# DeepLearningZ/chanamq

Measured on AMD Instinct MI355X. Metric: msgs/sec (whole node) + p50 publish→deliver latency, 1 KB payload, 1/2/4/8 GPUs, higher is better.
Workload: dtype uint8 (AMQP wire bytes; no floating-point compute)

## Files before the change

### csrc/kernels/dataplane.hip

```cpp
#include "dp_state.h"

#define INVALID 0xffffffffu
#define FNV64_BASIS 0xcbf29ce484222325ULL
#define FNV64_PRIME 0x100000001b3ULL

DEV u32 lane_id() { return __lane_id(); }
DEV u64 lanemask_lt() {
  u32 l = __lane_id();
  return l ? ((~0ull) >> (64 - l)) : 0ull;
}
DEV u32 be16(const u8* p) { return (u32(p[0]) << 8) | u32(p[1]); }
DEV u32 be32(const u8* p) {
  return (u32(p[0]) << 24) | (u32(p[1]) << 16) | (u32(p[2]) << 8) | u32(p[3]);
}
DEV u64 be64(const u8* p) { return (u64(be32(p)) << 32) | u64(be32(p + 4)); }
DEV void wr16(u8* p, u32 v) { p[0] = u8(v >> 8); p[1] = u8(v); }
DEV void wr32(u8* p, u32 v) { p[0] = u8(v >> 24); p[1] = u8(v >> 16); p[2] = u8(v >> 8); p[3] = u8(v); }
DEV void wr64(u8* p, u64 v) { wr32(p, u32(v >> 32)); wr32(p + 4, u32(v)); }
DEV u32 align16(u32 x) { return (x + 15u) & ~15u; }

DEV u64 exch_hash(u32 vhost, const u8* name, u32 n) {
  u64 h = FNV64_BASIS ^ (u64(vhost) * 0x9E3779B97F4A7C15ULL);
  for (u32 i = 0; i < n; ++i) { h ^= name[i]; h *= FNV64_PRIME; }
  return h;
// ... 157 lines not shown
DEV void release_msg(const DS& d, u32 msg) {
  if (msg == INVALID) return;
  i32 old = atomicSub(&d.msgs[msg].refcnt, 1);
  if (old == 1) {
    MsgEnt& m = d.msgs[msg];
    if (m.log_off & COLD_BIT) {
      atomicAdd((unsigned long long*)&d.cold_live[((m.log_off & ~COLD_BIT) >> COLD_SEG_SHIFT) % COLD_SEGS],
                (unsigned long long)(-(i64)m.slot_bytes));
    } else if (m.log_off & SPILL_BIT) {
      spill_free(d, m.log_off, m.slot_bytes);
    } else {
      u64 blk = (m.log_off / d.log_block) % d.n_log_blocks;
      atomicAdd((unsigned long long*)&d.log_live[blk], (unsigned long long)(-(i64)m.slot_bytes));
      atomicAdd((unsigned long long*)d.live_bytes, (unsigned long long)(-(i64)m.slot_bytes));
    }
    u32 slot = atomicAdd(d.msg_free_top, 1u);
    d.msg_free[slot] = msg;
    atomicAdd(&d.ctr->n_freed, 1u);
  }
}

DEV void wave_release(const DS& d, u32 msg, bool valid) {
  bool freed = false, spilled = false;
  u64 blk = 0;
  i64 sb = 0;
  if (valid && msg != INVALID) {
    i32 old = atomicSub(&d.msgs[msg].refcnt, 1);
    if (old == 1) {
      freed = true;
      const u64 lo = d.msgs[msg].log_off;
      sb = d.msgs[msg].slot_bytes;
      spilled = (lo & (SPILL_BIT | COLD_BIT)) != 0;
      if (lo & COLD_BIT)
        atomicAdd((unsigned long long*)&d.cold_live[((lo & ~COLD_BIT) >> COLD_SEG_SHIFT) % COLD_SEGS],
                  (unsigned long long)(-sb));
      else if (spilled) spill_free(d, lo, (u32)sb);
      else blk = (lo / d.log_block) % d.n_log_blocks;
    }
  }
  u64 fm = __ballot(freed);
  if (!fm) return;
  u32 nf;
  u32 pos = wave_reserve(d.msg_free_top, freed, &nf);
  if (freed) d.msg_free[pos] = msg;
  i64 tot = wave_sum64(freed && !spilled ? sb : 0);
  if (lane_id() == __ffsll((unsigned long long)fm) - 1) {
    atomicAdd(&d.ctr->n_freed, nf);
    if (tot) atomicAdd((unsigned long long*)d.live_bytes, (unsigned long long)(-tot));
  }
  wave_add_i64(d.log_live, blk, -sb, freed && !spilled);
}

DEV u64 snowflake_id(u64 pos, u32 group) {
  const u64 ms = pos >> ID_SLOT_BITS;
  const u64 worker = (u64)(group & (1023 / ID_WORKERS)) * ID_WORKERS + ((pos >> 12) & (ID_WORKERS - 1));
  return (ms << 22) | (worker << 12) | (pos & 4095);
}

struct Words { u32 eff; u32 count; };
DEV Words words_of(const u8* s, u32 n) {
  Words w;
  if (n == 0) { w.eff = 0; w.count = 1; return w; }
  u32 e = n;
  while (e > 0 && s[e - 1] == '.') --e;
  w.eff = e;
  if (e == 0) { w.count = 0; return w; }
  u32 c = 1;
  for (u32 i = 0; i < e; ++i) c += (s[i] == '.');
  w.count = c;
  return w;
}
DEV u32 word_len(const u8* s, u32 off, u32 eff) {
  u32 i = off;
  while (i < eff && s[i] != '.') ++i;
  return i - off;
}
DEV bool word_eq(const u8* a, u32 al, const u8* b, u32 bl) {
  if (al != bl) return false;
  for (u32 i = 0; i < al; ++i)
    if (a[i] != b[i]) return false;
  return true;
}
DEV bool topic_match(const u8* pat, u32 plen, const u8* key, u32 klen, bool hash_wild) {
  Words pw = words_of(pat, plen), kw = words_of(key, klen);
  u32 pend = pw.eff + 1, kend = kw.eff + 1;
  u32 p = pw.count ? 0 : pend, k = kw.count ? 0 : kend;
  u32 sp = INVALID, sk = 0;
  while (k < kend) {
    u32 kl = word_len(key, k, kw.eff);
    if (p < pend) {
      u32 pl = word_len(pat, p, pw.eff);
      bool is_hash = hash_wild && pl == 1 && pat[p] == '#';
      bool is_star = pl == 1 && pat[p] == '*';
      if (is_hash) { p += pl + 1; sp = p; sk = k; continue; }
      if (is_star || word_eq(pat + p, pl, key + k, kl)) { p += pl + 1; k += kl + 1; continue; }
    }
    if (sp != INVALID) {
      sk += word_len(key, sk, kw.eff) + 1;
      k = sk;
      p = sp;
      continue;
    }
    return false;
  }
  while (p < pend) {
    u32 pl = word_len(pat, p, pw.eff);
    if (hash_wild && pl == 1 && pat[p] == '#') { p += pl + 1; continue; }
    return false;
  }
  return true;
}

struct DeltaHead { u32 nrec, ndirty, nchunk, pad; };
struct DeltaRec { u64 dst; u32 len; u32 chunk0; };
#define DELTA_REC_MAX 1024
DEV void apply_deltas(const DS& d, const u8* buf, u32 tid, u32 nt, DeltaRec* lrec) {
  const DeltaHead h = *(const DeltaHead*)buf;
  const DeltaRec* recs = (const DeltaRec*)(buf + sizeof(DeltaHead));
  const u32* dirty = (const u32*)(recs + h.nrec);
  const uint4* data = (const uint4*)((const u8*)dirty + ((4u * h.ndirty + 15u) & ~15u));
  for (u32 r = tid; r < h.nrec; r += nt) lrec[r] = recs[r];
  __syncthreads();
  for (u32 i = tid; i < h.nchunk; i += nt) {
    u32 lo = 0, hi = h.nrec;
    while (hi - lo > 1) {
      const u32 mid = (lo + hi) >> 1;
      if (lrec[mid].chunk0 <= i) lo = mid; else hi = mid;
    }
    const DeltaRec r = lrec[lo];
    const u32 off = (i - r.chunk0) * 16u;
    const u32 n = r.len - off < 16u ? r.len - off : 16u;
    const uint4 v = data[i];
    u8* dst = (u8*)(uintptr_t)(r.dst + off);
    const u32 w[4] = {v.x, v.y, v.z, v.w};
    if (((uintptr_t)dst & 3) == 0 && (n & 3) == 0) {
      for (u32 k = 0; k < n / 4; ++k) ((u32*)dst)[k] = w[k];
    } else {
      for (u32 k = 0; k < n; ++k) dst[k] = (u8)(w[k >> 2] >> (8 * (k & 3)));
    }
  }
  __syncthreads();
  for (u32 k = tid; k < h.ndirty; k += nt) {
    const u32 ch = dirty[k];
    if (atomicExch(&d.ch_dirty[ch], 1u) == 0) d.dirty_list[atomicAdd(d.n_dirty, 1u)] = ch;
  }
  __threadfence();
  __syncthreads();
}
__global__ __launch_bounds__(1024) void k_apply_deltas(DS d, const u8* buf) {
  __shared__ DeltaRec lrec[DELTA_REC_MAX];
  apply_deltas(d, buf, threadIdx.x, 1024, lrec);
}

__global__ __launch_bounds__(64) void k_h2d_wait(DS d) {
  const u64 sig = d.in->h2d_sig, sig2 = d.in->h2d_sig2;
  if (!sig) return;
  const u32 lim = d.in->h2d_polls ? d.in->h2d_polls : (1u << 24);
  if (threadIdx.x == 0)
    for (u32 it = 0; it < lim; ++it) {
      if (__hip_atomic_load((const i64*)sig, __ATOMIC_RELAXED, __HIP_MEMORY_SCOPE_SYSTEM) == 0 &&
          (!sig2 || __hip_atomic_load((const i64*)sig2, __ATOMIC_RELAXED, __HIP_MEMORY_SCOPE_SYSTEM) == 0))
        break;
      __builtin_amdgcn_s_sleep(4);
    }
  __syncthreads();
  __builtin_amdgcn_fence(__ATOMIC_ACQUIRE, "");
}

__global__ __launch_bounds__(1024) void k_stage(DS d) {
  __shared__ u32 lds[1024 / 64 + 1];
  __shared__ StepIn s_in;
  __shared__ DeltaRec lrec[DELTA_REC_MAX];
  const u32 tid = threadIdx.x;
  if (tid == 0) {
    s_in = *d.in_h;
    *d.in = s_in;
  }
  __syncthreads();
  if (s_in.delta_bytes) apply_deltas(d, d.delta_h, tid, 1024, lrec);
  const u32 nseg = s_in.nseg;
  {
    u32* c = (u32*)d.ctr;
    for (u32 k = tid; k < sizeof(Counters) / 4; k += 1024)
      if (k * 4 < offsetof(Counters, log_head)) c[k] = 0;
    if (tid == 0) {
      d.ctr->n_grow = 0; d.tot[TS_NMOVE] = 0; d.tot[TS_NDEFER] = 0; d.tot[TS_TTL_BUDGET] = 0;
      d.tot[TS_NDGET] = 0;
      d.tot[TS_SPILL_USED] = 0;
      d.ctr->spill_moved = 0;
      d.ctr->n_ref = 0; d.ctr->gath_off = 0; d.ctr->ref_bytes = 0;
      *d.egress_budget = 0;
    }
    const u32 nunp = s_in.nunp;
    for (u32 k = tid; k < nunp; k += 1024) {
      const u32 c = d.unpause_req[k];
      if (c < d.c_max) d.conn_paused[c] = 0;
    }
  }
  u32 total = 0;
  u32 cl0 = 0, len0 = 0;
  for (u32 k = tid; k < nseg; k += 1024) {
    const SegIn sg = d.segs_h[k];
    ((SegIn*)d.segs)[k] = sg;
    const u32 cl = d.carry_len[sg.conn];
    if (k == tid) { cl0 = cl; len0 = sg.len; }
    total += align16(cl + sg.len + 32);
  }
  u32 all_t;
  block_scan<1024>(total, lds, all_t);
  if (tid == 0) d.tot[15] = all_t;
  if (all_t > d.work_cap) return;
  u32 run = 0;
  for (u32 b0 = 0; b0 < nseg; b0 += 1024) {
    const u32 k = b0 + tid;
    u32 cl = 0, len = 0, v = 0;
    if (k < nseg) {
      if (b0 == 0) {
        cl = cl0;
        len = len0;
      } else {
        const SegIn sg = d.segs_h[k];
        cl = d.carry_len[sg.conn];
        len = sg.len;
      }
      v = align16(cl + len + 32);
    }
    u32 all;
    __syncthreads();
    const u32 o = block_scan<1024>(v, lds, all);
    if (k < nseg) { d.seg_total[k] = cl + len; d.seg_start[k] = run + o; }
    run += all;
  }
}

struct FInfo { u32 type, ch, size; bool complete, valid_hdr; };

DEV FInfo frame_at(const u8* b, u32 p, u32 L, u32 fmax) {
  FInfo f;
  f.complete = false;
  f.valid_hdr = false;
  f.type = 0; f.ch = 0; f.size = 0;
  if (p + 7 > L) return f;
  f.type = b[p];
  f.ch = be16(b + p + 1);
  f.size = be32(b + p + 3);
  bool tok = f.type == 1 || f.type == 2 || f.type == 3 || f.type == 8;
  bool sok = fmax == 0 || f.size + 8 <= fmax;
  f.valid_hdr = tok && sok;
  if (f.valid_hdr && (u64)p + 8 + f.size <= L) f.complete = (b[p + 7 + f.size] == 0xCE);
  return f;
}

DEV i32 chan_lookup(const DS& d, u32 conn, u32 ch) {
  const u32* m = d.chmap + (u64)conn * d.chmap_size;
  u32 mask = d.chmap_size - 1;
  u32 h = (ch * 0x9E3779B1u) >> 7;
  for (u32 i = 0; i < d.chmap_size; ++i) {
    u32 e = m[(h + i) & mask];
    if (e == 0) return -1;
    if ((e >> 16) == ch && (e & 0x8000u)) return (i32)(conn * d.chpc + (e & 0x7fffu));
  }
  return -1;
}

DEV u32 zero_bytes(u32 v) { return ~(((v & 0x7F7F7F7Fu) + 0x7F7F7F7Fu) | v | 0x7F7F7F7Fu); }
DEV u32 type_nibble(u32 v) {
  const u32 h = (zero_bytes(v & 0xFCFCFCFCu) & ~zero_bytes(v)) | zero_bytes(v ^ 0x08080808u);
  return (((h >> 7) * 0x00204081u) >> 21) & 0xFu;
}
DEV u32 cand_bits(uint4 A, uint4 B, u32 fm) {
  const u32 w[6] = {A.x, A.y, A.z, A.w, B.x, B.y};
  u32 m = 0;
#pragma unroll
  for (int i = 0; i < 4; ++i) {
    u32 h = type_nibble(w[i]);
    while (h) {
      const u32 k = __ffs(h) - 1;
      h &= h - 1;
      const u32 v = k == 0 ? __builtin_amdgcn_alignbyte(w[i + 1], w[i], 3)
                           : __builtin_amdgcn_alignbyte(w[i + 2], w[i + 1], k - 1);
      const u32 sz = __builtin_bswap32(v);
      if (fm == 0 || sz <= fm - 8) m |= 1u << (4 * i + k);
    }
  }
  return m;
}
DEV u32 cand_word(const u8* w16, u32 fm) {
  const uint4* q = (const uint4*)w16;
  return cand_bits(q[0], q[1], fm);
}

#define FS_MARK(k) \
  do { if (tid == 0 && d.dbg) d.dbg[(u64)s * 16 + (k)] = __builtin_amdgcn_s_memrealtime(); } while (0)
constexpr u32 FS_AM_MAX = 8192;
constexpr u32 FS_STAGE = 72u << 10;
constexpr u32 FS_CAND_STAGED = 6144;
constexpr u32 fs_cand_bytes(u32 cmax, u32 amw) { return cmax * 4 * 2 + (cmax > amw ? cmax : amw) * 2 + cmax * 2 + cmax; }
constexpr u32 FS_POOL_STAGED = FS_STAGE + fs_cand_bytes(FS_CAND_STAGED, FS_STAGE / 16);
constexpr u32 FS_POOL_FULL = fs_cand_bytes(CAND_MAX, FS_AM_MAX);
constexpr u32 FS_POOL = ((FS_POOL_STAGED > FS_POOL_FULL ? FS_POOL_STAGED : FS_POOL_FULL) + 15) & ~15u;
static_assert(FS_POOL <= 156u << 10, "k_frame_scan LDS pool");
#define FS_NT 1024
DEV bool big_publish(const DS& d, u32 msize, u32 hsize, u64 bsz, u32 fmax) {
  const u64 fb = fmax > 8 ? fmax - 8 : 0;
  const u64 nb = bsz == 0 ? 0 : (fb ? (bsz + fb - 1) / fb : 1);
  return (u64)msize + 8 + hsize + 8 + bsz + 8 * nb > d.carry_cap;
}

DEV uint4 shift_pair(uint4 a, uint4 b, u32 sh) {
  const u32 q = sh >> 2, r = sh & 3;
  const bool q2 = (q & 2) != 0, q1 = (q & 1) != 0;
  const u32 s0 = q2 ? a.z : a.x, s1 = q2 ? a.w : a.y, s2 = q2 ? b.x : a.z;
  const u32 s3 = q2 ? b.y : a.w, s4 = q2 ? b.z : b.x, s5 = q2 ? b.w : b.y;
  const u32 w0 = q1 ? s1 : s0, w1 = q1 ? s2 : s1, w2 = q1 ? s3 : s2, w3 = q1 ? s4 : s3, w4 = q1 ? s5 : s4;
  if (!r) return make_uint4(w0, w1, w2, w3);
  return make_uint4(__builtin_amdgcn_alignbyte(w1, w0, r), __builtin_amdgcn_alignbyte(w2, w1, r),
                    __builtin_amdgcn_alignbyte(w3, w2, r), __builtin_amdgcn_alignbyte(w4, w3, r));
}
DEV uint4 seg_word(const u8* C, u32 cl, const u8* N, u32 c) {
  const u32 b0 = c * 16;
  if (b0 + 16 <= cl) return *(const uint4*)(C + b0);
  if (b0 >= cl) {
    const u32 o = b0 - cl, k = o >> 4, sh = o & 15;
    const uint4 a = ((const uint4*)N)[k];
    return sh ? shift_pair(a, ((const uint4*)N)[k + 1], sh) : a;
  }
// ... 2126 lines not shown
}
DEV u32 enqueue_one(const DS& d, u32 src, u32 i, u32 n, PersistRec* pr, u32 hs_ntiles) {
  const u32* kk = d.pair_k[src];
  const u32 rb = d.rank_bits;
  u32 q = kk[i] >> rb;
  u32 p = d.pair_v[src][i];
  u32 first = hs_ntiles ? d.hist_scan[q << rb] : d.q_first[q];
  return enqueue_at(d, q, p, i - first, (i + 1 == n) || (kk[i + 1] >> rb) != q, pr);
}

DEV void plan_queue(const DS& d, u32 q, u64 cnt);
DEV void ring_plan_one(const DS& d, u32 src, u32 hs_ntiles, u32 i, u32 n) {
  const u32* kk = d.pair_k[src];
  const u32 rb = d.rank_bits;
  const u32 q = kk[i] >> rb;
  if (i + 1 < n && (kk[i + 1] >> rb) == q) return;
  const u32 first = hs_ntiles ? d.hist_scan[q << rb] : d.q_first[q];
  plan_queue(d, q, (u64)(i - first) + 1);
}
DEV void plan_queue(const DS& d, u32 q, u64 cnt) {
  const u64 head = d.q_head[q], tail = d.q_tail[q];
  d.q_enq_tail[q] = tail;
  const u64 mask = d.q_ring_mask[q], cap = mask + 1;
  const u64 need = tail - head + cnt;
  if (need <= cap) return;
  const u64 limit = d.q_max_cap[q] ? d.q_max_cap[q] : d.ring_pool;
  u64 want = cap;
  while (want < 2 * need && want * 2 <= limit) want *= 2;
  if (want <= cap) return;
  unsigned long long* top = (unsigned long long*)d.ring_top;
  u64 off = __hip_atomic_load(top, __ATOMIC_RELAXED, __HIP_MEMORY_SCOPE_AGENT);
  while (true) {
    if (off + want > d.ring_pool) return;
    u64 prev = atomicCAS(top, off, off + want);
    if (prev == off) break;
    off = prev;
  }
  RingMove mv;
  mv.q = q; mv.pad = 0;
  mv.old_off = d.q_ring_off[q]; mv.old_mask = mask;
  mv.new_off = off; mv.new_mask = want - 1;
  mv.head = head; mv.tail = tail;
  const u32 mi = atomicAdd(&d.tot[TS_NMOVE], 1u);
  d.moves[mi] = mv;
  d.q_ring_off[q] = off;
  d.q_ring_mask[q] = want - 1;
  const u32 gi = atomicAdd(&d.ctr->n_grow, 1u);
  if (gi < GROW_MAX) d.grow_h[gi] = mv;
  __threadfence();
}

__global__ __launch_bounds__(256) void k_ring_plan(DS d, u32 src, u32 hs_ntiles) {
  __shared__ u32 s_last;
  const u32 n = d.tot[TS_PAIR_N];
  u32 nb = (n + 255) / 256;
  if (nb > gridDim.x) nb = gridDim.x;
  if (blockIdx.x >= nb) return;
  for (u32 i = blockIdx.x * 256 + threadIdx.x; i < n; i += gridDim.x * 256) ring_plan_one(d, src, hs_ntiles, i, n);
  __builtin_amdgcn_fence(__ATOMIC_RELEASE, "workgroup");
  __syncthreads();
  if (threadIdx.x == 0) s_last = atomicAdd(&d.tot[TS_RP_TICKET], 1u) == nb - 1;
  __syncthreads();
  if (!s_last) return;
  __builtin_amdgcn_fence(__ATOMIC_ACQUIRE, "agent");
  if (threadIdx.x == 0) d.tot[TS_RP_TICKET] = 0;
  const u32 nm = d.tot[TS_NMOVE];
  for (u32 m = 0; m < nm; ++m) {
    const RingMove mv = d.moves[m];
    for (u64 pos = mv.head + threadIdx.x; pos < mv.tail; pos += 256)
      d.ring[mv.new_off + (pos & mv.new_mask)] = d.ring[mv.old_off + (pos & mv.old_mask)];
  }
}

__global__ void k_enqueue(DS d, u32 src, u32 hs_ntiles) {
  const u32 n = d.tot[TS_PAIR_N];
  const u32 stride = gridDim.x * blockDim.x;
  for (u32 b = blockIdx.x * blockDim.x; b < n; b += stride) {
    const u32 i = b + threadIdx.x;
    PersistRec pr;
    pr.msg = INVALID;
    u32 drop = i < n ? enqueue_one(d, src, i, n, &pr, hs_ntiles) : INVALID;
    wave_release(d, drop, drop != INVALID);
    if (drop != INVALID) atomicAdd(&d.ctr->n_ring_full, 1u);
    if (d.persist) {
      bool want = pr.msg != INVALID;
      u32 k = wave_reserve(&d.ctr->n_persist, want);
      if (want && k < d.persist_max) d.prec[k] = pr;
    }
  }
}

DEV void plan_rings_block(const DS& d, const u32* hscan, u32 n, u32 D, u32 tid, u32 nt) {
  const u32 rb = d.rank_bits;
  for (u32 q = tid; q < d.q_max && (q << rb) < D; q += nt) {
    const u32 first = __hip_atomic_load(&hscan[q << rb], __ATOMIC_RELAXED, __HIP_MEMORY_SCOPE_AGENT);
    const u32 nx = ((q + 1) << rb) < D
                       ? __hip_atomic_load(&hscan[(q + 1) << rb], __ATOMIC_RELAXED, __HIP_MEMORY_SCOPE_AGENT)
                       : n;
    if (nx > first) plan_queue(d, q, nx - first);
  }
  __syncthreads();
  const u32 nm = __hip_atomic_load(&d.tot[TS_NMOVE], __ATOMIC_RELAXED, __HIP_MEMORY_SCOPE_AGENT);
  if (!nm) return;
  __builtin_amdgcn_fence(__ATOMIC_ACQUIRE, "agent");
  for (u32 m = 0; m < nm; ++m) {
    const RingMove mv = d.moves[m];
    for (u64 pos = mv.head + tid; pos < mv.tail; pos += nt)
      d.ring[mv.new_off + (pos & mv.new_mask)] = d.ring[mv.old_off + (pos & mv.old_mask)];
  }
}

template <int DB>
__global__ __launch_bounds__(RsNt<DB>::v) void k_rs_hist_plan(DS d, const u32* keys, const u32* np, u32* hist,
                                                             u32* hscan, u32* ticket, u32 ntiles) {
  constexpr u32 NT = RsNt<DB>::v, D = 1u << DB;
  __shared__ u32 cnt[D];
  __shared__ u32 lds[NT / 64 + 1];
  __shared__ u32 s_last;
  u32 tid = threadIdx.x, t = blockIdx.x;
  const u32 n = *np;
  u32 T = (n + SORT_TILE - 1) / SORT_TILE;
  if (T > ntiles) T = ntiles;
  if (T == 0) {
    return;
  }
  if (t >= T) return;
  bool last = false;
  for (; t < T; t += gridDim.x) {
    for (u32 k = tid; k < D; k += NT) cnt[k] = 0;
    __syncthreads();
    const u32 base = t * SORT_TILE;
    for (u32 j = 0; j < SORT_TILE / NT; ++j) {
      const u32 i = base + j * NT + tid;
      if (i < n) atomicAdd(&cnt[keys[i] & (D - 1)], 1u);
    }
    __syncthreads();
    for (u32 k = tid; k < D; k += NT)
      __hip_atomic_store(&hist[t * D + k], cnt[k], __ATOMIC_RELAXED, __HIP_MEMORY_SCOPE_AGENT);
    __builtin_amdgcn_fence(__ATOMIC_RELEASE, "workgroup");
    __syncthreads();
    if (tid == 0) s_last = atomicAdd(ticket, 1u) == T - 1;
    __syncthreads();
    last = last || s_last;
  }
  if (!last) return;
  __builtin_amdgcn_fence(__ATOMIC_ACQUIRE, "agent");
  if (tid == 0) *ticket = 0;
  rs_offsets<DB>(hist, hscan, T, lds);
  __builtin_amdgcn_fence(__ATOMIC_RELEASE, "workgroup");
  __syncthreads();
  plan_rings_block(d, hscan, n, D, tid, NT);
}

template <int DB>
__global__ __launch_bounds__(256) void k_rs_scatter_enq(DS d, const u32* kin, const u32* vin, const u32* np,
                                                       const u32* hscan) {
  constexpr u32 D = 1u << DB, CH = SORT_TILE / 256;
  __shared__ u32 wc[4][D];
  const u32 tid = threadIdx.x, w = tid >> 6, lane = tid & 63;
  const u32 n = *np, rb = d.rank_bits;
  const u64 lt = lanemask_lt();
  for (u32 t = blockIdx.x; t * SORT_TILE < n; t += gridDim.x) {
    const u32 base = t * SORT_TILE;
    __syncthreads();
    for (u32 i = tid; i < 4 * D; i += 256) ((u32*)wc)[i] = 0;
    __syncthreads();
    const u32 wbase = base + w * (SORT_TILE / 4);
    u32 key[CH], val[CH];
    u64 pe[CH];
#pragma unroll
    for (u32 c = 0; c < CH; ++c) {
      const u32 i = wbase + c * 64 + lane;
      key[c] = i < n ? kin[i] : 0u;
      val[c] = i < n ? vin[i] : 0u;
    }
#pragma unroll
    for (u32 c = 0; c < CH; ++c) {
      const bool valid = wbase + c * 64 + lane < n;
      const u32 dg = key[c] & (D - 1);
      u64 peers = __ballot(valid);
#pragma unroll
      for (u32 bb = 0; bb < DB; ++bb) {
        const u64 m = __ballot((dg >> bb) & 1);
        peers &= ((dg >> bb) & 1) ? m : ~m;
      }
      pe[c] = peers;
      if (valid && ((peers & lt) == 0)) wc[w][dg] += __popcll(peers);
      __builtin_amdgcn_wave_barrier();
    }
    __syncthreads();
    for (u32 dg = tid; dg < D; dg += 256) {
      u32 run = hscan[t * D + dg];
      for (u32 ww = 0; ww < 4; ++ww) { const u32 x = wc[ww][dg]; wc[ww][dg] = run; run += x; }
    }
    __syncthreads();
    u32 pos[CH];
#pragma unroll
    for (u32 c = 0; c < CH; ++c) {
      const bool valid = wbase + c * 64 + lane < n;
      const u32 dg = key[c] & (D - 1);
      const u32 basepos = ((volatile u32*)wc[w])[dg];
      pos[c] = basepos + __popcll(pe[c] & lt);
      __builtin_amdgcn_wave_barrier();
      if (valid && ((pe[c] & lt) == 0)) ((volatile u32*)wc[w])[dg] = basepos + __popcll(pe[c]);
      __builtin_amdgcn_wave_barrier();
    }
    EnqLoad el[CH];
    u32 first[CH], nx[CH];
#pragma unroll
    for (u32 c = 0; c < CH; ++c) {
      const bool valid = wbase + c * 64 + lane < n;
      const u32 q = key[c] >> rb;
      first[c] = valid ? hscan[q << rb] : 0u;
      nx[c] = valid ? (((q + 1) << rb) < D ? hscan[(q + 1) << rb] : n) : 0u;
      el[c] = valid ? enq_load(d, q, val[c]) : EnqLoad{};
    }
#pragma unroll
    for (u32 c = 0; c < CH; ++c) {
      const bool valid = wbase + c * 64 + lane < n;
      PersistRec pr;
      pr.msg = INVALID;
      u32 drop = INVALID;
      if (valid) drop = enq_store(d, el[c], key[c] >> rb, pos[c] - first[c], pos[c] + 1 == nx[c], &pr);
      wave_release(d, drop, drop != INVALID);
      if (drop != INVALID) atomicAdd(&d.ctr->n_ring_full, 1u);
      if (d.persist) {
        const bool want = pr.msg != INVALID;
        const u32 k = wave_reserve(&d.ctr->n_persist, want);
        if (want && k < d.persist_max) d.prec[k] = pr;
      }
    }
  }
}

DEV bool wants_record(const DS& d, u32 msg, u32 q, bool valid) {
  return d.persist && valid && msg != INVALID && d.q_durable[q] && (d.msgs[msg].flags & MF_PERSIST);
}
DEV void consumed_rec_at(const DS& d, u32 msg, u32 q, u64 qpos, u32 kind, u32 k) {
  ConsumedRec r;
  r.msg_id = (i64)d.msgs[msg].msg_id;
  r.qpos = qpos;
  r.q = q;
  r.kind = kind;
  r.pad[0] = r.pad[1] = 0;
  d.crec[k] = r;
}
DEV void link_consumed(const DS& d, u32 msg, u32 q, u32 kind, bool valid) {
  if (d.links && valid && msg != INVALID && kind <= 2u) {
    const u32 ow = d.q_link_owner[q];
    if (ow) {
      const u32 k = atomicAdd(&d.lk_cnt[ow - 1], 1u);
      if (k < d.lk_cap) {
        AckRec a;
        a.tq = q;
        a.pad = 0;
        a.xid = d.msgs[msg].msg_id;
        d.lk_send[(u64)(ow - 1) * d.lk_cap + k] = a;
      }
    }
  }
}
DEV void wave_consumed(const DS& d, u32 msg, u32 q, u64 qpos, u32 kind, bool valid) {
  link_consumed(d, msg, q, kind, valid);
  if (!d.persist) return;
  bool want = wants_record(d, msg, q, valid);
  u32 k = wave_reserve(&d.ctr->n_consumed, want);
  if (want && k < d.persist_max) consumed_rec_at(d, msg, q, qpos, kind, k);
}


#define MS_MAX 256
struct MsLds {
  u64 up[MS_MAX];
  u32 rq[MS_MAX];
  u32 wc[4];
  u32 rc[4];
  u32 rbase;
  u32 n, nb;
  unsigned long long ovf_a, ovf_r;
};
DEV void chan_advance_one(const DS& d, u32 ch, u32 tid, u32 lane, u32 w, u32* s_first, u32* s_done, MsLds& ms);
__global__ __launch_bounds__(256) void k_chan_advance(DS d) {
  __shared__ u32 s_first[4];
  __shared__ u32 s_done[4];
  __shared__ MsLds ms;
  const u32 tid = threadIdx.x, lane = lane_id(), w = tid >> 6;
  const u32 nd = *d.n_dirty;
  for (u32 wv = blockIdx.x; wv < nd; wv += gridDim.x) chan_advance_one(d, d.dirty_list[wv], tid, lane, w, s_first,
                                                                        s_done, ms);
}

DEV void collect_settles(const DS& d, u32 ch, u32 tid, u32 lane, u32 w, MsLds& ms) {
  const u32 lo = d.ch_mlo[ch], hi = d.ch_mhi[ch];
  if (tid == 0) { ms.n = 0; ms.nb = 0; ms.ovf_a = 0; ms.ovf_r = 0; }
  __syncthreads();
  if (lo == INVALID) return;
  for (u32 base = lo; base <= hi; base += 256) {
    const u32 i = base + tid;
    bool take = false;
    Ack a;
    a.tag = 0; a.kind = 0; a.requeue = 0;
    if (i <= hi) {
      a = d.acks[i];
      take = a.chslot == ch && a.multiple;
    }
    const bool rq = (a.kind != CK_ACK) && a.requeue;
    const u64 m = __ballot(take);
    if (lane == 0) ms.wc[w] = (u32)__popcll(m);
    __syncthreads();
    u32 pos = ms.n + (u32)__popcll(m & lanemask_lt());
    for (u32 k = 0; k < w; ++k) pos += ms.wc[k];
    if (take) {
      if (pos < MS_MAX) { ms.up[pos] = a.tag; ms.rq[pos] = rq; }
      else atomicMax(rq ? &ms.ovf_r : &ms.ovf_a, (unsigned long long)a.tag);
    }
    __syncthreads();
    if (tid == 0) ms.n += ms.wc[0] + ms.wc[1] + ms.wc[2] + ms.wc[3];
    __syncthreads();
  }
  if (tid == 0) {
    const u32 n = ms.n < MS_MAX ? ms.n : MS_MAX;
    u64 top = 0;
    u32 nb = 0;
    for (u32 k = 0; k < n; ++k)
      if (ms.up[k] > top) { ms.up[nb] = ms.up[k]; ms.rq[nb] = ms.rq[k]; ++nb; top = ms.up[k]; }
    const u64 oa = ms.ovf_a, orq = ms.ovf_r;
    const u64 om = oa > orq ? oa : orq;
    if (om > top && nb < MS_MAX) { ms.up[nb] = om; ms.rq[nb] = orq > oa; ++nb; }
    ms.nb = nb;
    d.ch_mlo[ch] = INVALID;
    d.ch_mhi[ch] = 0;
  }
  __syncthreads();
}

DEV u32 ca_reserve(const DS& d, u32 n) {
  const u32 lim = d.persist_max - d.deliv_max - (d.persist_max >> 2) - 64u;
  u32 cur = *(volatile u32*)&d.ctr->n_consumed;
  while (true) {
    if (cur + n > lim) return INVALID;
    const u32 prev = atomicCAS(&d.ctr->n_consumed, cur, cur + n);
    if (prev == cur) return cur;
    cur = prev;
  }
}

DEV void chan_advance_one(const DS& d, u32 ch, u32 tid, u32 lane, u32 w, u32* s_first, u32* s_done, MsLds& ms) {
  collect_settles(d, ch, tid, lane, w, ms);
  const u32 nb = ms.nb;
  const u64 head = d.ch_uhead[ch], nt = d.ch_next_tag[ch];
  const u64 aup = d.ch_ack_upto[ch], rup = d.ch_req_upto[ch];
  USlot* win = d.uwin + (u64)ch * (d.ucap_mask + 1);
  bool contiguous = true;
  bool deferred = false;
  u64 newhead = head;
  u32 manual_done = 0;
  for (u64 t0 = head; t0 < nt; t0 += 256) {
    const u64 t = t0 + tid;
    const bool valid = t < nt;
    u32 st = US_FREE;
    USlot u;
    u.state = US_FREE; u.msg = INVALID; u.q = 0; u.cons = 0; u.qpos = 0; u.expire_ms = 0;
    if (valid) {
      u = win[(t - 1) & d.ucap_mask];
      st = u.state;
      if (st == US_PENDING) {
        if (t <= aup) st = US_ACKED;
        else if (t <= rup) st = US_REQUEUE;
        else
          for (u32 k = 0; k < nb; ++k)
            if (t <= ms.up[k]) { st = ms.rq[k] ? US_REQUEUE : US_ACKED; break; }
      }
    }
    const bool acked = valid && st == US_ACKED;
    const bool req = valid && st == US_REQUEUE;
    u32 rec_k = INVALID;
    const bool want_rec = wants_record(d, u.msg, u.q, acked || req);
    if (d.persist) {
      const u64 rm = __ballot(want_rec);
      if (lane == 0) ms.rc[w] = (u32)__popcll(rm);
      __syncthreads();
      if (tid == 0) {
        const u32 tot = ms.rc[0] + ms.rc[1] + ms.rc[2] + ms.rc[3];
        ms.rbase = deferred ? INVALID : (tot ? ca_reserve(d, tot) : 0u);
      }
      __syncthreads();
      if (ms.rbase == INVALID) deferred = true;
      if (!deferred) {
        rec_k = ms.rbase + (u32)__popcll(rm & lanemask_lt());
        for (u32 k = 0; k < w; ++k) rec_k += ms.rc[k];
      }
    }
    if (deferred) {
      if (valid && (st == US_ACKED || st == US_REQUEUE) && st != u.state) win[(t - 1) & d.ucap_mask].state = st;
      contiguous = false;
      continue;
    }
    u32 rtot;
    u32 ri = wave_reserve(d.req_n, req, &rtot);
    bool req_ok = req && ri < d.req_max;
    if (req_ok) {
      ReqItem r;
      r.q = u.q; r.msg = u.msg; r.qpos = u.qpos; r.expire_ms = u.expire_ms;
      d.req[ri] = r;
    }
    wave_add_u32(d.req_q_n, u.q, 1u, req_ok);
    link_consumed(d, u.msg, u.q, acked ? 0u : (req_ok ? 4u : 2u), acked || req);
    if (want_rec) consumed_rec_at(d, u.msg, u.q, u.qpos, acked ? 0u : (req_ok ? 4u : 2u), rec_k);
    wave_release(d, u.msg, acked || (req && !req_ok));
    wave_sub_u32(d.cons_unacked, u.cons, 1u, acked || req);
    manual_done += __popcll(__ballot(acked || req));
    if (lane == 0 && rtot) atomicAdd(&d.ctr->n_requeue, rtot);
    if (acked || req) st = US_DONE;
    if (valid && st != u.state) win[(t - 1) & d.ucap_mask].state = st;
    if (contiguous) {
      const u64 notdone = __ballot(valid && st != US_DONE);
      const u32 nvalid = (u32)__popcll(__ballot(valid));
      if (lane == 0) {
        s_first[w] = notdone ? (u32)(__ffsll((unsigned long long)notdone) - 1) : 64u;
        s_done[w] = nvalid;
      }
      __syncthreads();
      u32 adv = 0;
      bool stop = false;
      for (u32 k = 0; k < 4 && !stop; ++k) {
        if (s_first[k] < 64) { adv += s_first[k]; stop = true; }
        else adv += s_done[k];
      }
      newhead += adv;
      if (stop) contiguous = false;
      __syncthreads();
    }
  }
  if (lane == 0 && manual_done) atomicSub(&d.ch_unacked[ch], manual_done);
// ... 1548 lines not shown
```

### csrc/kernels/engine.hip

```cpp
#include <pybind11/pybind11.h>
#include <pybind11/numpy.h>
#include <pybind11/stl.h>

#include <chrono>
#include <algorithm>
#include <deque>
#include <functional>
#include <map>
#include <memory>
#include <mutex>
#include <condition_variable>
#include <thread>
#include <stdexcept>
#include <string>
#include <vector>

#include <hsa/amd_hsa_signal.h>
#include <hsa/hsa.h>
#include <hsa/hsa_ext_amd.h>
#include <rocprofiler-sdk-roctx/roctx.h>

#include "dataplane.hip"
#include "xchg_host.h"
#include "xchg_rccl.h"
// ... 2158 lines not shown
      if (t == HSA_DEVICE_TYPE_GPU) c->gpus.push_back(a);
      else if (t == HSA_DEVICE_TYPE_CPU) c->cpus.push_back(a);
      return HSA_STATUS_SUCCESS;
    }, &ctx);
    if ((int)ctx.gpus.size() <= device_ || ctx.cpus.empty()) throw std::runtime_error("HSA agents not found");
    {
      u64 f = 0;
      if (hsa_system_get_info(HSA_SYSTEM_INFO_TIMESTAMP_FREQUENCY, &f) != HSA_STATUS_SUCCESS || !f) f = 100000000ull;
      spin_ticks_ = f / 500;
      block_ticks_ = f / 1000;
    }
    gpu_agent_ = ctx.gpus[device_];
    cpu_agent_ = ctx.cpus[0];
    uint32_t mask = 0;
    if (hsa_amd_memory_copy_engine_status(cpu_agent_, gpu_agent_, &mask) != HSA_STATUS_SUCCESS || !mask)
      throw std::runtime_error("no SDMA engine available for device -> host copies");
    u32 pick = 0;
    if (sdma_pref_ >= 0 && (mask >> sdma_pref_) & 1u) pick = (u32)sdma_pref_;
    else if ((mask >> 1) & 1u) pick = 1;
    else while (!((mask >> pick) & 1u)) ++pick;
    sdma_engine_ = (hsa_amd_sdma_engine_id_t)(1u << pick);
    sdma_engine2_ = (hsa_amd_sdma_engine_id_t)0;
    if (sdma_split_ > 1)
      for (u32 c : {2u, 3u, 0u})
        if (c != pick && ((mask >> c) & 1u)) { sdma_engine2_ = (hsa_amd_sdma_engine_id_t)(1u << c); break; }
    tail_engine_ = sdma_engine_;
    for (u32 c : {2u, 3u, 0u})
      if (c != pick && ((mask >> c) & 1u) && (1u << c) != (u32)sdma_engine2_) {
        tail_engine_ = (hsa_amd_sdma_engine_id_t)(1u << c);
        break;
      }
    ing_engine_ = (hsa_amd_sdma_engine_id_t)0;
    for (u32 c : {0u, 3u, 2u, 1u})
      if (((mask >> c) & 1u) && (1u << c) != (u32)sdma_engine_ && (1u << c) != (u32)sdma_engine2_ &&
          (1u << c) != (u32)tail_engine_) {
        ing_engine_ = (hsa_amd_sdma_engine_id_t)(1u << c);
        break;
      }
    if (!ing_engine_) ing_engine_ = tail_engine_;
    ing_engine2_ = (hsa_amd_sdma_engine_id_t)0;
    if (h2d_split_cfg_)
      for (u32 c : {3u, 2u})
        if (((mask >> c) & 1u) && (1u << c) != (u32)ing_engine_ && (1u << c) != (u32)sdma_engine_ &&
            (1u << c) != (u32)sdma_engine2_ && (1u << c) != (u32)tail_engine_) {
          ing_engine2_ = (hsa_amd_sdma_engine_id_t)(1u << c);
          break;
        }
    for (int e = 0; e < EGRESS_SLOTS; ++e)
      if (hsa_signal_create(0, 0, nullptr, &sdma_sig_[e]) != HSA_STATUS_SUCCESS ||
          hsa_signal_create(0, 0, nullptr, &tail_sig_[e]) != HSA_STATUS_SUCCESS ||
          hsa_signal_create(0, 0, nullptr, &gate_sig_[e]) != HSA_STATUS_SUCCESS)
        throw std::runtime_error("hsa_signal_create failed");
  }

  void drain_egress() {
    for (int e = 0; e < EGRESS_SLOTS; ++e) {
      sdma_wait(e);
      if (d2h_issued_[e]) HIPCHECK(hipEventSynchronize(ev_d2h_[e]));
    }
  }

  void sync() {
    HIPCHECK(hipStreamSynchronize(s_h2d_));
    if (s_h2d_alt_) HIPCHECK(hipStreamSynchronize(s_h2d_alt_));
    HIPCHECK(hipStreamSynchronize(s_pre_));
    HIPCHECK(hipStreamSynchronize(s_ing_));
    HIPCHECK(hipStreamSynchronize(s_comp_));
    HIPCHECK(hipStreamSynchronize(s_d2h_));
  }

  py::dict host_times(bool reset) {
    static const char* names[9] = {"submit", "submit_sdma_wait", "submit_graph_launch", "wait_results",
                                   "egress_copy", "egress_wait", "exchange", "exchange_counts", "exchange_thread"};
    py::dict o;
    for (int i = 0; i < 9; ++i) { o[names[i]] = ht_[i]; if (reset) ht_[i] = 0; }
    return o;
  }

  py::dict counters(int p) const {
    const Counters& c = *(const Counters*)buf("ctr_host" + std::to_string(p)).ptr;
    py::dict o;
#define F(x) o[#x] = c.x
    F(n_cmds); F(n_frags); F(n_pubs); F(n_acks); F(n_ctrl); F(ctrl_bytes); F(n_pairs); F(n_deliv);
    F(egress_bytes); F(n_returns); F(n_confirm_frames); F(n_freed); F(n_requeue); F(n_unroutable);
    F(n_dropped_nomem); F(n_expired); F(n_routed_msgs); F(n_unknown_exchange); F(n_ring_full);
    F(n_acked); F(log_head); F(log_tail); F(msg_free_top); F(n_live_msgs);
    F(n_persist); F(n_consumed); F(persist_used); F(n_persist_overflow);
    F(live_bytes); F(n_grow); F(n_dget); F(spill_moved); F(n_ref); F(gath_off); F(ref_bytes);
#undef F
    std::vector<u32> lat(c.lat_hist, c.lat_hist + LAT_BINS);
    o["lat_hist"] = lat;
    return o;
  }

 private:
  static ScanArgs scan_args(std::initializer_list<std::pair<const u32*, u32*>> arrs, const u32* n, u32 nmax,
                            u32 slot, const u32* lo) {
    if (arrs.size() > 4) throw std::runtime_error("launch_scan: at most 4 arrays");
    ScanArgs a{};
    a.lo = lo;
    u32 k = 0;
    for (auto& p : arrs) { a.in[k] = p.first; a.out[k] = p.second; ++k; }
    a.narr = k;
    a.n = n;
    a.nmax = nmax;
    a.tot_slot = slot;
    return a;
  }
  void launch_scan(hipStream_t s, const DS& d, std::initializer_list<std::pair<const u32*, u32*>> arrs, const u32* n,
                   u32 nmax, u32 slot, const u32* lo = nullptr, bool ingest = false) {
    const ScanArgs a = scan_args(arrs, n, nmax, slot, lo);
    u32 nb = ceil_div(nmax ? nmax : 1, SCAN_TILE);
    hipLaunchKernelGGL((k_scan<4, 4>), dim3(nb), dim3(1024), 0, s, a, d.tot, ingest ? scan_status_ing_ : scan_status_,
                       ingest ? scan_ctl_ing_ : scan_ctl_, scan_smax_);
  }
  u32 radix_sort(hipStream_t s, const DS& d, u32** keys, u32** vals, const u32* n, u32 nmax, u32 bits) {
    u32 ntiles = ceil_div(nmax, SORT_TILE);
    if (bits > 8 && bits <= 11) {
      if (bits == 9) {
        hipLaunchKernelGGL(k_rs_hist<9>, capped(ntiles, 256), dim3(RsNt<9>::v), 0, s, keys[0], n, 0u, d_.hist,
                           d_.hist_scan, &d.tot[TS_RS_TICKET], ntiles);
        hipLaunchKernelGGL(k_rs_scatter<9>, capped(ntiles, 256), dim3(256), 0, s, keys[0], vals[0], keys[1], vals[1], n,
                           0u, d_.hist_scan, ntiles);
      } else if (bits == 10) {
        hipLaunchKernelGGL(k_rs_hist<10>, capped(ntiles, 256), dim3(RsNt<10>::v), 0, s, keys[0], n, 0u, d_.hist,
                           d_.hist_scan, &d.tot[TS_RS_TICKET], ntiles);
        hipLaunchKernelGGL(k_rs_scatter<10>, capped(ntiles, 256), dim3(256), 0, s, keys[0], vals[0], keys[1], vals[1],
                           n, 0u, d_.hist_scan, ntiles);
      } else {
        hipLaunchKernelGGL(k_rs_hist<11>, capped(ntiles, 256), dim3(RsNt<11>::v), 0, s, keys[0], n, 0u, d_.hist,
                           d_.hist_scan, &d.tot[TS_RS_TICKET], ntiles);
        hipLaunchKernelGGL(k_rs_scatter<11>, capped(ntiles, 256), dim3(256), 0, s, keys[0], vals[0], keys[1], vals[1],
                           n, 0u, d_.hist_scan, ntiles);
      }
      return 1;
    }
    u32 src = 0;
    for (u32 shift = 0; shift < bits; shift += 8) {
      hipLaunchKernelGGL(k_rs_hist<8>, capped(ntiles, 256), dim3(RsNt<8>::v), 0, s, keys[src], n, shift, d_.hist, d_.hist_scan,
                         &d.tot[TS_RS_TICKET], ntiles);
      hipLaunchKernelGGL(k_rs_scatter<8>, capped(ntiles, 256), dim3(256), 0, s, keys[src], vals[src], keys[src ^ 1],
                         vals[src ^ 1], n, shift, d_.hist_scan, ntiles);
      src ^= 1;
    }
    return src;
  }

  static dim3 blocks(u64 n, u32 per) { return dim3(n ? ceil_div(n, per) : 1); }
  static dim3 wave_blocks(u64 n) { u64 b = n ? ceil_div(n, 4) : 1; return dim3(b > 8192 ? 8192 : (u32)b); }
  static dim3 capped(u64 b, u32 cap) { return dim3(b == 0 ? 1u : (b > cap ? cap : (u32)b)); }

  void launch_ingest(hipStream_t s, const DS& d) {
    Range rg("chanamq.K1-K4.ingest");
    hipLaunchKernelGGL(k_stage, dim3(1), dim3(1024), 0, s, d);
    if (h2d_hsa_) hipLaunchKernelGGL(k_h2d_wait, dim3(16), dim3(64), 0, s, d);
    hipLaunchKernelGGL(k_frame_scan, capped(d.seg_max, n_cu_), dim3(FS_NT), 0, s, d);
    if (d.rank_scan)
      launch_scan(s, d, {{d.cmd_is_pub, d.cmd_pub_rank}, {d.cmd_is_ack, d.cmd_ack_rank}}, &d.ctr->n_cmds,
                  d.cmd_max, 4, nullptr, true);
    hipLaunchKernelGGL(k_decode, blocks(d.cmd_max, 256), dim3(256), 0, s, d);
  }

  void launch_route(hipStream_t s, const DS& d, u32 nmax, bool imports = false) {
    Range rg("chanamq.K6-K13.route_store");
    const u64 ngroups = ceil_div(nmax ? nmax : 1, 16);
    if (imports) hipLaunchKernelGGL(k_import_route, capped(ngroups, n_cu_), dim3(1024), 0, s, d);
    else hipLaunchKernelGGL(k_route, capped(ngroups, 2 * n_cu_), dim3(1024), 0, s, d);
    const ScanArgs a = scan_args({{d.pub_nq, d.pub_pair_off}, {d.pub_slot, d.pub_slot_off},
                                  {d.pub_routed, d.pub_routed_rank}, {d.pub_ret_sz, d.pub_ret_off}},
                                 &d.tot[TS_RANGE_HI], d.pub_cap, 0, &d.tot[TS_RANGE_LO]);
    hipLaunchKernelGGL(k_scan_route, dim3(ceil_div(d.pub_cap ? d.pub_cap : 1, SCAN_TILE)), dim3(1024), 0, s, a, d.tot,
                       scan_status_, scan_ctl_, scan_smax_, d);
    hipLaunchKernelGGL(k_route_store, wave_blocks(nmax), dim3(256), 0, s, d, imports ? 0u : 1u);
  }

  void launch_pack(hipStream_t s, const DS& d) {
    Range rg("chanamq.X1.pack");
    hipLaunchKernelGGL(k_pack_scan, blocks(d.pub_max, PK_TILE), dim3(1024), 0, s, d, d.pk_agg, &d.tot[TS_PK_TICKET]);
    hipLaunchKernelGGL(k_pack, wave_blocks(d.pub_max), dim3(256), 0, s, d);
  }

  void launch_tail(hipStream_t s, const DS& d, bool dispatch = true) {
    Range rg("chanamq.K7-K11.tail");
    u32 nch = d.c_max * d.chpc;
    const u32 pbits = d.q_bits + d.rank_bits;
    if (pbits <= 11) {
      const u32 nt = ceil_div(d.pair_max, SORT_TILE);
      const u32* n = &d.tot[TS_PAIR_N];
      u32* tk = &d.tot[TS_RS_TICKET];
      if (pbits <= 8) {
        hipLaunchKernelGGL(k_rs_hist_plan<8>, capped(nt, 256), dim3(RsNt<8>::v), 0, s, d, d.pair_k[0], n, d_.hist, d_.hist_scan, tk, nt);
        hipLaunchKernelGGL(k_rs_scatter_enq<8>, capped(nt, 256), dim3(256), 0, s, d, d.pair_k[0], d.pair_v[0], n, d_.hist_scan);
      } else if (pbits == 9) {
        hipLaunchKernelGGL(k_rs_hist_plan<9>, capped(nt, 256), dim3(RsNt<9>::v), 0, s, d, d.pair_k[0], n, d_.hist, d_.hist_scan, tk, nt);
        hipLaunchKernelGGL(k_rs_scatter_enq<9>, capped(nt, 256), dim3(256), 0, s, d, d.pair_k[0], d.pair_v[0], n, d_.hist_scan);
      } else if (pbits == 10) {
        hipLaunchKernelGGL(k_rs_hist_plan<10>, capped(nt, 256), dim3(RsNt<10>::v), 0, s, d, d.pair_k[0], n, d_.hist, d_.hist_scan, tk, nt);
        hipLaunchKernelGGL(k_rs_scatter_enq<10>, capped(nt, 256), dim3(256), 0, s, d, d.pair_k[0], d.pair_v[0], n, d_.hist_scan);
      } else {
        hipLaunchKernelGGL(k_rs_hist_plan<11>, capped(nt, 256), dim3(RsNt<11>::v), 0, s, d, d.pair_k[0], n, d_.hist, d_.hist_scan, tk, nt);
        hipLaunchKernelGGL(k_rs_scatter_enq<11>, capped(nt, 256), dim3(256), 0, s, d, d.pair_k[0], d.pair_v[0], n, d_.hist_scan);
      }
    } else {
      u32* pk[2] = {d.pair_k[0], d.pair_k[1]};
      u32* pv[2] = {d.pair_v[0], d.pair_v[1]};
      const u32 psrc = radix_sort(s, d, pk, pv, &d.tot[TS_PAIR_N], d.pair_max, pbits);
      hipLaunchKernelGGL(k_qfirst, blocks(d.pair_max, 256), dim3(256), 0, s, d, psrc);
      hipLaunchKernelGGL(k_ring_plan, capped(ceil_div(d.pair_max, 256), 1024), dim3(256), 0, s, d, psrc, 0u);
      hipLaunchKernelGGL(k_enqueue, capped(ceil_div(d.pair_max, 256), 1024), dim3(256), 0, s, d, psrc, 0u);
    }
    const u32 fin = d.persist ? 0u : 1u;
    if (!dispatch) {
      const u64 pn = d.deliv_max > d.c_max ? d.deliv_max : d.c_max;
      hipLaunchKernelGGL(k_post, blocks(pn, 256), dim3(256), 0, s, d, fin);
      if (!fin) hipLaunchKernelGGL(k_host_out, dim3(64), dim3(256), 0, s, d);
      return;
    }
    hipLaunchKernelGGL(k_chan_advance, capped(nch, 1024), dim3(256), 0, s, d);
    hipLaunchKernelGGL(k_dequeue, dim3(d.q_max), dim3(256), 0, s, d);
    hipLaunchKernelGGL(k_dv_write, blocks(d.deliv_max, 256), dim3(256), 0, s, d);
    if (d.c_max <= CONN_LAYOUT_MAX) {
      hipLaunchKernelGGL(k_conn_layout, dim3(1), dim3(1024), 0, s, d);
    } else {
      launch_scan(s, d, {{d.dv_size, d.dv_off}}, &d.ctr->n_deliv, d.deliv_max, 6);
      hipLaunchKernelGGL(k_conn_sizes, blocks(d.c_max, 256), dim3(256), 0, s, d);
      launch_scan(s, d, {{d.conn_total, d.conn_base}}, nullptr, d.c_max, 7);
      hipLaunchKernelGGL(k_conn_out, blocks(d.c_max, 256), dim3(256), 0, s, d);
    }
    if (d.links) hipLaunchKernelGGL(k_link_bases, dim3(1), dim3(64), 0, s, d);
    {
      const u32 n_rc = RC_RET_BLOCKS + ceil_div(d.c_max, 256);
      hipLaunchKernelGGL(k_render, dim3(n_rc + wave_blocks(d.deliv_max).x), dim3(256), 0, s, d, n_rc);
    }
    u64 pn = d.deliv_max > d.c_max ? d.deliv_max : d.c_max;
    hipLaunchKernelGGL(k_post, blocks(pn, 256), dim3(256), 0, s, d, fin);
    if (d.persist) {
      hipLaunchKernelGGL(k_persist_size, blocks(d.persist_max, 256), dim3(256), 0, s, d);
      launch_scan(s, d, {{d.ps_size, d.ps_off}}, &d.ctr->n_persist, d.persist_max, TS_PERSIST);
      hipLaunchKernelGGL(k_persist_pack, wave_blocks(d.persist_max), dim3(256), 0, s, d);
      hipLaunchKernelGGL(k_host_out, dim3(64), dim3(256), 0, s, d);
    }
  }

  void launch_main(hipStream_t s, const DS& d) {
    launch_ingest(s, d);
    launch_route(s, d, d.pub_max);
    if (d.world > 1) launch_pack(s, d);
    else launch_tail(s, d);
  }

  void launch_rest(hipStream_t s, const DS& d) {
    launch_route(s, d, d.pub_max);
    launch_tail(s, d);
  }
  void capture_on(hipStream_t st, hipGraphExec_t* ge, const std::function<void()>& f) {
    hipGraph_t g;
    std::lock_guard<std::mutex> cg(cap_mu_);
    HIPCHECK(hipStreamBeginCapture(st, hipStreamCaptureModeThreadLocal));
    f();
    HIPCHECK(hipStreamEndCapture(st, &g));
    HIPCHECK(hipGraphInstantiate(ge, g, nullptr, nullptr, 0));
    HIPCHECK(hipGraphDestroy(g));
  }

  void launch_phase_b(hipStream_t s, const DS& d, bool dispatch = true) {
    Range rg("chanamq.X1.import");
    launch_route(s, d, d.import_max, true);
    launch_tail(s, d, dispatch);
  }

  void capture_main(int p) {
    hipGraph_t g;
    std::lock_guard<std::mutex> cg(cap_mu_);
    HIPCHECK(hipStreamBeginCapture(s_comp_, hipStreamCaptureModeThreadLocal));
    launch_main(s_comp_, io_[p]);
    HIPCHECK(hipStreamEndCapture(s_comp_, &g));
    HIPCHECK(hipGraphInstantiate(&graph_exec_[p], g, nullptr, nullptr, 0));
    HIPCHECK(hipGraphDestroy(g));
  }

  void capture_b(int p) {
    hipGraph_t g;
    std::lock_guard<std::mutex> cg(cap_mu_);
    HIPCHECK(hipStreamBeginCapture(s_comp_, hipStreamCaptureModeThreadLocal));
    launch_phase_b(s_comp_, io_[p]);
    HIPCHECK(hipStreamEndCapture(s_comp_, &g));
    HIPCHECK(hipGraphInstantiate(&graph_b_[p], g, nullptr, nullptr, 0));
    HIPCHECK(hipGraphDestroy(g));
  }

  int device_ = 0;
  u32 n_cu_ = 256;
  DS d_;
  std::map<std::string, Buf> bufs_;
  u64 total_bytes_ = 0;
  u64 egress_alloc_ = 0;
  int ref_back_ = -1;
  u32 ref_min_ = 256;
  u32 ntiles_max_ = 0;
  u32 restore_max_ = 0;
  u64 carry_budget_ = 0;
  u64 get_cap_ = 0;
  u8* get_out_dev_ = nullptr;
  GetRes* get_res_dev_ = nullptr;
  u64* scan_status_ = nullptr;
  unsigned long long* spill_moved_ = nullptr;
  u32* scan_ctl_ = nullptr;
  u32 scan_smax_ = 0;
  bool graph_enabled_ = true;
  bool sdma_ = true;
  hipGraphExec_t graph_exec_[NPAR_MAX] = {};
  hipGraphExec_t graph_b_[NPAR_MAX] = {};
  hipEvent_t ev_a_[NPAR_MAX], ev_ext_[NPAR_MAX];
  bool phase_a_[NPAR_MAX] = {};
  bool counts_ready_[NPAR_MAX] = {};
  bool lag_ = false;
  std::vector<u32> lag_recv_;
  u64 lag_stream_ = 0;
  bool xfer_set_ = false;
  bool native_x_ = false;
  bool b_due_[NPAR_MAX] = {};
  std::unique_ptr<cmqx::RcclXchg> rccl_;
  std::unique_ptr<cmqx::ShmXchg> shm_;
  std::unique_ptr<cmqx::ShmXchg> cshm_;
  std::vector<int> xmembers_;
  int xtimeout_ms_ = 10000;
  bool xfailover_ = false;
  bool x_wait_ = false;
  u64 xseq_ = 0;
  bool async_x_ = false;
  std::thread xth_;
  std::mutex xmu_;
  std::condition_variable xcv_;
  bool xstop_ = false, xjob_ = false, xbusy_ = false, xres_ = false;
  int xq_ = 0, xres_rc_ = 0;
  u32 xflags_ = 0, xres_orf_ = 0, xjob_seq_ = 0, xseq_job_ = 0;
  std::string xerr_;
  u32 b_wait_[NPAR_MAX] = {};
  u32* xflag_h_ = nullptr;
  std::mutex cap_mu_;
  hipStream_t s_x_ = nullptr;
  std::mutex io_mu_;
  hipStream_t s_io_ = nullptr;
  u32* xflag_d_ = nullptr;
  u8* xs_desc_[2] = {nullptr, nullptr};
  u8* xs_pay_[2] = {nullptr, nullptr};
  u8* xr_desc_[2] = {nullptr, nullptr};
  u8* xr_pay_[2] = {nullptr, nullptr};
  bool links_ = false;
  u8* ls_desc_[2] = {nullptr, nullptr};
  u8* ls_pay_[2] = {nullptr, nullptr};
  u8* lk_send_[2] = {nullptr, nullptr};
  u8* rack_[2] = {nullptr, nullptr};
  struct HostIO : DS {
    const Counters* ctr_host_h = nullptr;
    const SegOut* seg_out_hh = nullptr;
    const ConnOut* conn_out_hh = nullptr;
    const CtrlRec* ctrl_rec_hh = nullptr;
    const u8* ctrl_hh = nullptr;
    const u8* persist_hh = nullptr;
    const ConsumedRec* crec_hh = nullptr;
    const RingMove* grow_hh = nullptr;
    const u32* conn_conf_hh = nullptr;
    const GetOut* get_out_hh = nullptr;
  };
  std::vector<GetReq> pend_gets_;
  static constexpr u64 DELTA_CAP = 4ull << 20;
  std::mutex dl_mu_;
  struct DlBatch { std::map<u64, std::string> w; std::vector<u32> dirty, unp; u64 bytes = 0; bool open = false; u64 id = 0; };
  std::vector<u32> unp_ready_;
  u32 spill_req_[3] = {0, 0, 0};
// ... 265 lines not shown
```

Before: 49.04 million.

## Fold h2d wait into k_stage and chan_advance into scatter_enq launch

```diff
diff --git a/csrc/kernels/dataplane.hip b/csrc/kernels/dataplane.hip
--- a/csrc/kernels/dataplane.hip
+++ b/csrc/kernels/dataplane.hip
@@ -333,26 +333,30 @@
   apply_deltas(d, buf, threadIdx.x, 1024, lrec);
 }
 
-__global__ __launch_bounds__(64) void k_h2d_wait(DS d) {
-  const u64 sig = d.in->h2d_sig, sig2 = d.in->h2d_sig2;
+DEV void h2d_wait_wave(const StepIn* in) {
+  const u64 sig = in->h2d_sig, sig2 = in->h2d_sig2;
   if (!sig) return;
-  const u32 lim = d.in->h2d_polls ? d.in->h2d_polls : (1u << 24);
-  if (threadIdx.x == 0)
+  const u32 lim = in->h2d_polls ? in->h2d_polls : (1u << 24);
+  if (lane_id() == 0)
     for (u32 it = 0; it < lim; ++it) {
       if (__hip_atomic_load((const i64*)sig, __ATOMIC_RELAXED, __HIP_MEMORY_SCOPE_SYSTEM) == 0 &&
           (!sig2 || __hip_atomic_load((const i64*)sig2, __ATOMIC_RELAXED, __HIP_MEMORY_SCOPE_SYSTEM) == 0))
         break;
       __builtin_amdgcn_s_sleep(4);
     }
-  __syncthreads();
   __builtin_amdgcn_fence(__ATOMIC_ACQUIRE, "");
 }
+#define STAGE_WAIT_BLOCKS 16
 
 __global__ __launch_bounds__(1024) void k_stage(DS d) {
   __shared__ u32 lds[1024 / 64 + 1];
   __shared__ StepIn s_in;
   __shared__ DeltaRec lrec[DELTA_REC_MAX];
   const u32 tid = threadIdx.x;
+  if (blockIdx.x > 0) {
+    if (tid < 64) h2d_wait_wave(d.in_h);
+    return;
+  }
   if (tid == 0) {
     s_in = *d.in_h;
     *d.in = s_in;
@@ -2785,15 +2789,36 @@
   plan_rings_block(d, hscan, n, D, tid, NT);
 }
 
+#define MS_MAX 256
+struct MsLds {
+  u64 up[MS_MAX];
+  u32 rq[MS_MAX];
+  u32 wc[4];
+  u32 rc[4];
+  u32 rbase;
+  u32 n, nb;
+  unsigned long long ovf_a, ovf_r;
+};
+DEV void chan_advance_one(const DS& d, u32 ch, u32 tid, u32 lane, u32 w, u32* s_first, u32* s_done, MsLds& ms);
 template <int DB>
 __global__ __launch_bounds__(256) void k_rs_scatter_enq(DS d, const u32* kin, const u32* vin, const u32* np,
-                                                       const u32* hscan) {
+                                                       const u32* hscan, u32 n_ca) {
   constexpr u32 D = 1u << DB, CH = SORT_TILE / 256;
   __shared__ u32 wc[4][D];
   const u32 tid = threadIdx.x, w = tid >> 6, lane = tid & 63;
+  const u32 nenq = gridDim.x - n_ca;
+  if (blockIdx.x >= nenq) {
+    __shared__ u32 s_first[4];
+    __shared__ u32 s_done[4];
+    __shared__ MsLds ms;
+    const u32 nd = *d.n_dirty;
+    for (u32 wv = blockIdx.x - nenq; wv < nd; wv += n_ca)
+      chan_advance_one(d, d.dirty_list[wv], tid, lane, w, s_first, s_done, ms);
+    return;
+  }
   const u32 n = *np, rb = d.rank_bits;
   const u64 lt = lanemask_lt();
-  for (u32 t = blockIdx.x; t * SORT_TILE < n; t += gridDim.x) {
+  for (u32 t = blockIdx.x; t * SORT_TILE < n; t += nenq) {
     const u32 base = t * SORT_TILE;
     __syncthreads();
     for (u32 i = tid; i < 4 * D; i += 256) ((u32*)wc)[i] = 0;
@@ -2902,17 +2927,6 @@
 }
 
 
-#define MS_MAX 256
-struct MsLds {
-  u64 up[MS_MAX];
-  u32 rq[MS_MAX];
-  u32 wc[4];
-  u32 rc[4];
-  u32 rbase;
-  u32 n, nb;
-  unsigned long long ovf_a, ovf_r;
-};
-DEV void chan_advance_one(const DS& d, u32 ch, u32 tid, u32 lane, u32 w, u32* s_first, u32* s_done, MsLds& ms);
 __global__ __launch_bounds__(256) void k_chan_advance(DS d) {
   __shared__ u32 s_first[4];
   __shared__ u32 s_done[4];
diff --git a/csrc/kernels/engine.hip b/csrc/kernels/engine.hip
--- a/csrc/kernels/engine.hip
+++ b/csrc/kernels/engine.hip
@@ -2334,8 +2334,7 @@
 
   void launch_ingest(hipStream_t s, const DS& d) {
     Range rg("chanamq.K1-K4.ingest");
-    hipLaunchKernelGGL(k_stage, dim3(1), dim3(1024), 0, s, d);
-    if (h2d_hsa_) hipLaunchKernelGGL(k_h2d_wait, dim3(16), dim3(64), 0, s, d);
+    hipLaunchKernelGGL(k_stage, dim3(1 + (h2d_hsa_ ? STAGE_WAIT_BLOCKS : 0)), dim3(1024), 0, s, d);
     hipLaunchKernelGGL(k_frame_scan, capped(d.seg_max, n_cu_), dim3(FS_NT), 0, s, d);
     if (d.rank_scan)
       launch_scan(s, d, {{d.cmd_is_pub, d.cmd_pub_rank}, {d.cmd_is_ack, d.cmd_ack_rank}}, &d.ctr->n_cmds,
@@ -2370,18 +2369,19 @@
       const u32 nt = ceil_div(d.pair_max, SORT_TILE);
       const u32* n = &d.tot[TS_PAIR_N];
       u32* tk = &d.tot[TS_RS_TICKET];
+      const u32 n_ca = dispatch ? capped(nch, 1024).x : 0u;
       if (pbits <= 8) {
         hipLaunchKernelGGL(k_rs_hist_plan<8>, capped(nt, 256), dim3(RsNt<8>::v), 0, s, d, d.pair_k[0], n, d_.hist, d_.hist_scan, tk, nt);
-        hipLaunchKernelGGL(k_rs_scatter_enq<8>, capped(nt, 256), dim3(256), 0, s, d, d.pair_k[0], d.pair_v[0], n, d_.hist_scan);
+        hipLaunchKernelGGL(k_rs_scatter_enq<8>, dim3(capped(nt, 256).x + n_ca), dim3(256), 0, s, d, d.pair_k[0], d.pair_v[0], n, d_.hist_scan, n_ca);
       } else if (pbits == 9) {
         hipLaunchKernelGGL(k_rs_hist_plan<9>, capped(nt, 256), dim3(RsNt<9>::v), 0, s, d, d.pair_k[0], n, d_.hist, d_.hist_scan, tk, nt);
-        hipLaunchKernelGGL(k_rs_scatter_enq<9>, capped(nt, 256), dim3(256), 0, s, d, d.pair_k[0], d.pair_v[0], n, d_.hist_scan);
+        hipLaunchKernelGGL(k_rs_scatter_enq<9>, dim3(capped(nt, 256).x + n_ca), dim3(256), 0, s, d, d.pair_k[0], d.pair_v[0], n, d_.hist_scan, n_ca);
       } else if (pbits == 10) {
         hipLaunchKernelGGL(k_rs_hist_plan<10>, capped(nt, 256), dim3(RsNt<10>::v), 0, s, d, d.pair_k[0], n, d_.hist, d_.hist_scan, tk, nt);
-        hipLaunchKernelGGL(k_rs_scatter_enq<10>, capped(nt, 256), dim3(256), 0, s, d, d.pair_k[0], d.pair_v[0], n, d_.hist_scan);
+        hipLaunchKernelGGL(k_rs_scatter_enq<10>, dim3(capped(nt, 256).x + n_ca), dim3(256), 0, s, d, d.pair_k[0], d.pair_v[0], n, d_.hist_scan, n_ca);
       } else {
         hipLaunchKernelGGL(k_rs_hist_plan<11>, capped(nt, 256), dim3(RsNt<11>::v), 0, s, d, d.pair_k[0], n, d_.hist, d_.hist_scan, tk, nt);
-        hipLaunchKernelGGL(k_rs_scatter_enq<11>, capped(nt, 256), dim3(256), 0, s, d, d.pair_k[0], d.pair_v[0], n, d_.hist_scan);
+        hipLaunchKernelGGL(k_rs_scatter_enq<11>, dim3(capped(nt, 256).x + n_ca), dim3(256), 0, s, d, d.pair_k[0], d.pair_v[0], n, d_.hist_scan, n_ca);
       }
     } else {
       u32* pk[2] = {d.pair_k[0], d.pair_k[1]};
@@ -2398,7 +2398,7 @@
       if (!fin) hipLaunchKernelGGL(k_host_out, dim3(64), dim3(256), 0, s, d);
       return;
     }
-    hipLaunchKernelGGL(k_chan_advance, capped(nch, 1024), dim3(256), 0, s, d);
+    if (pbits > 11) hipLaunchKernelGGL(k_chan_advance, capped(nch, 1024), dim3(256), 0, s, d);
     hipLaunchKernelGGL(k_dequeue, dim3(d.q_max), dim3(256), 0, s, d);
     hipLaunchKernelGGL(k_dv_write, blocks(d.deliv_max, 256), dim3(256), 0, s, d);
     if (d.c_max <= CONN_LAYOUT_MAX) {
```

Result: no change. 49.06 million, median of 5 (+0.0%).
